# amberxie88/latent_diffusion_planning

Hardware: AMD Instinct MI355X
Metric: latent plans/sec (horizon=9, 100 DDIM steps) (higher is better)
Workload: dtype f32; 1 GPU; configs[1]: rm_lift planner ConditionalUnet1D (D=25, T=8, down_dims [256,512,1024]), 100-step DDIM, batch 256 synthetic latents per GPU, random-init weights, Philox noise, hipGraph-captured loop; plans_per_gpu=256, denoise_steps=100, sampler=ddim, graph=True, parallelism=dp1, ranks_seen_by_backend=1, backend=none, range_fallback=0, fp16_plane_launches=0

## Files before the change

### latent_diffusion_planning_amd/csrc/engine.hip

```cpp
#include "engine.hpp"
#include "sconv.hpp"
#include "t2pack.hpp"
#include "t4pack.hpp"
#include "version.h"

#include <algorithm>
#include <cmath>
#include <cstring>

namespace ldp {

void betas_squaredcos(int n, std::vector<float>& betas, std::vector<float>& alphas,
                             std::vector<float>& acp) {
  auto abar = [](double t) {
    const double c = std::cos((t + 0.008) / 1.008 * M_PI / 2.0);
    return c * c;
  };
  betas.resize(n);
  alphas.resize(n);
  acp.resize(n);
  float run = 1.0f;
  for (int i = 0; i < n; ++i) {
    const double b = std::min(1.0 - abar((double)(i + 1) / n) / abar((double)i / n), 0.999);
    betas[i] = (float)b;
// ... 145 lines not shown
            const uint16_t mm = f32_to_bf16_rne(r1);
            const float r2 = r1 - bf16_to_f32(mm);
            dst[0 * 512 + lane * 8 + e] = hh;
            dst[1 * 512 + lane * 8 + e] = mm;
            dst[2 * 512 + lane * 8 + e] = f32_to_bf16_rne(r2);
          }
      }
  return p;
}

bool fits_f16_planes(const float* w, size_t n) {
  for (size_t i = 0; i < n; ++i)
    if (!(std::fabs(w[i]) < 65504.0f)) return false;
  return true;
}

static int split_tile(int to, bool res_out) {
  if (to == 2) return 32;
  if (to == 8 || to == 4) return 16;
  return 0;
}

static bool split_tile_updown(int mode, int to, int cout) {
  const int bn = cout / 8;
  if (mode == MODE_DOWN) return (to == 4 && (bn == 32 || bn == 64)) || (to == 2 && bn == 64);
  if (mode == MODE_UP) return (to == 4 && bn == 64) || (to == 8 && (bn == 32 || bn == 64)) || (to == 16 && bn == 32);
  return false;
}

static bool t2_cs2_ok(const ldp_handle* h, int B, int cout) {
  const int wgs = ((B + 31) / 32) * 8;
  return h->opt.planner_split_cs2 && !h->opt.no_csplit && !h->safe_mode && cout % 512 == 0 && 2 * wgs <= h->n_cu && 8 * wgs >= 3 * h->n_cu;
}

static int split_tile_at(const ldp_handle* h, int B, int to, bool res_out, int cout) {
  int tile = split_tile(to, res_out);
  if (to == 16 && cout == 256 && !res_out && h->f16_planner() && h->opt.planner_split_t16) tile = 16;
  if (cout % 256 != 0 || (cout == 256 && (tile == 32 || h->opt.planner_split_c256 == 0))) return 0;
  if (tile == 32) {
    const int wgs = ((B + 31) / 32) * 8;
    const bool filled = wgs >= h->n_cu || h->opt.planner_split >= 2;
    if (!filled) {
      const bool cs2 = t2_cs2_ok(h, B, cout);
      const bool whole16 = h->opt.planner_split_t2res16 && h->opt.planner_split_t2all16 && h->f16_planner() && cout % 512 == 0 && B > 256;
      tile = (cs2 || whole16) ? 33 : 0;
    }
  }
  return tile;
}

int get_weight(ldp_handle* h, const std::string& path, const HostTensor** out,
               std::initializer_list<int64_t> shape) {
  auto it = h->weights.find(path);
  if (it == h->weights.end()) return fail(LDP_ESTATE, "weight '%s' was never set", path.c_str());
  const HostTensor& t = it->second;
  if (t.shape.size() != shape.size() || !std::equal(shape.begin(), shape.end(), t.shape.begin())) {
    std::string got, want;
    for (auto s : t.shape) got += std::to_string(s) + ",";
    for (auto s : shape) want += std::to_string(s) + ",";
    return fail(LDP_EINVAL, "weight '%s' has shape (%s) expected (%s)", path.c_str(), got.c_str(),
                want.c_str());
  }
  *out = &t;
  return LDP_OK;
}

static int upload_padded(DevBuf& dst, const float* src, int n, int n_p, float fill, hipStream_t s) {
  std::vector<float> tmp(n_p, fill);
  std::copy(src, src + n, tmp.begin());
  LDP_TRY(dst.alloc((size_t)n_p * 4));
  LDP_HIP(hipMemcpy(dst.p, tmp.data(), (size_t)n_p * 4, hipMemcpyHostToDevice));
  (void)s;
  return LDP_OK;
}

int make_conv(ldp_handle* h, const std::string& prefix, int nj, int cin, int cout, int cin_p,
              int cout_p, const char* gn_prefix, hipStream_t s, ConvW& out, int t_pos) {
  const HostTensor *k = nullptr, *b = nullptr;
  LDP_TRY(get_weight(h, prefix + "/kernel", &k, {nj, cin, cout}));
  LDP_TRY(get_weight(h, prefix + "/bias", &b, {cout}));
  out.t2s = nj == 5 && t2_shared(MODE_K5, t_pos, 0);
  out.t4s = nj == 5 && t4_shared(MODE_K5, t_pos, 0);
  std::vector<float> packed = out.t2s ? pack_conv_t2(k->data.data(), nullptr, cin, cout, cin_p, cout_p)
                            : out.t4s ? pack_conv_t4(k->data.data(), nullptr, cin, cout, cin_p, cout_p)
                                      : pack_conv(k->data.data(), nj, cin, cout, cin_p, cout_p);
  LDP_TRY(out.w.alloc(packed.size() * 4));
  LDP_HIP(hipMemcpy(out.w.p, packed.data(), packed.size() * 4, hipMemcpyHostToDevice));
  LDP_TRY(upload_padded(out.bias, b->data.data(), cout, cout_p, 0.f, s));
  out.nj = nj; out.cin = cin; out.cout = cout; out.cin_p = cin_p; out.cout_p = cout_p;
  out.has_gn = gn_prefix != nullptr;
  out.wsplit.release(); out.wsplit16.release(); out.wsplit16h.release(); out.wsplith.release();
  out.f16_refused = false;
  if (gn_prefix) {
    const HostTensor *gs = nullptr, *gb = nullptr;
    LDP_TRY(get_weight(h, std::string(gn_prefix) + "/scale", &gs, {cout}));
    LDP_TRY(get_weight(h, std::string(gn_prefix) + "/bias", &gb, {cout}));
    LDP_TRY(upload_padded(out.gn_scale, gs->data.data(), cout, cout_p, 1.f, s));
    LDP_TRY(upload_padded(out.gn_bias, gb->data.data(), cout, cout_p, 0.f, s));
  }
  return LDP_OK;
}

static int add_res_proj(ldp_handle* h, const std::string& conv_prefix, const std::string& prefix, int cin,
                        int cout, int cin_p, ConvW& c) {
  const HostTensor *k = nullptr, *b = nullptr, *kc = nullptr;
  LDP_TRY(get_weight(h, prefix + "/kernel", &k, {1, cin, cout}));
  LDP_TRY(get_weight(h, prefix + "/bias", &b, {cout}));
  LDP_TRY(get_weight(h, conv_prefix + "/kernel", &kc, {c.nj, cin, cout}));
  c.wsplit.release(); c.wsplit16.release(); c.wsplit16h.release(); c.wsplith.release();
  c.f16_refused = false;
  std::vector<float> packed;
  if (c.t2s) {
    packed = pack_conv_t2(kc->data.data(), k->data.data(), cin, cout, cin_p, c.cout_p);
  } else if (c.t4s) {
    packed = pack_conv_t4(kc->data.data(), k->data.data(), cin, cout, cin_p, c.cout_p);
  } else {
    std::vector<float> both(kc->data);
    both.insert(both.end(), k->data.begin(), k->data.end());
    packed = pack_conv(both.data(), c.nj + 1, cin, cout, cin_p, c.cout_p);
  }
  LDP_TRY(c.w.alloc(packed.size() * 4));
  LDP_HIP(hipMemcpy(c.w.p, packed.data(), packed.size() * 4, hipMemcpyHostToDevice));
  LDP_TRY(c.bres.alloc((size_t)cout * 4));
  LDP_HIP(hipMemcpy(c.bres.p, b->data.data(), (size_t)cout * 4, hipMemcpyHostToDevice));
  c.has_res = true;
  return LDP_OK;
}

static int round_up(int v, int m) { return (v + m - 1) / m * m; }

static int pick_plan(int mode, int to, int cout, int cin_total, int ca, bool res_out, ConvPlan& p,
                     int* cs_io = nullptr, int mb_want = 1, bool up_full_depth = false) {
  const int gw = cout >= 256 ? cout / 8 : 32;
  if (cs_io && *cs_io == 4) {
    const int qb = gw / 4;
    int ks4 = 0, cpi4 = 0;
    if (mode == MODE_K5) {
      if (to == 2 && qb == 32) { ks4 = 4; cpi4 = 2; }
      else if (to == 4 && qb == 16) { ks4 = 8; cpi4 = 1; }
      else if (to == 8 && qb == 16) { ks4 = 8; cpi4 = 1; }
      else if (to == 4 && qb == 32) { ks4 = 4; cpi4 = res_out ? 1 : 2; }
    }
    const int chunk4 = 16 * ks4 * cpi4;
    if (ks4 && cin_total % chunk4 == 0 && ca % chunk4 == 0) {
      p = ConvPlan{mode, to, qb / 16, ks4, cpi4, res_out ? 1 : 0};
      return LDP_OK;
    }
    *cs_io = 2;
  }
  if (cs_io && *cs_io == 2) {
    const int hb = gw / 2;
    int ks2 = 0, cpi2 = 0;
    if (mode == MODE_K5) {
      if (to == 8 && hb == 16) { ks2 = (cin_total % 128 == 0) ? 8 : 4; cpi2 = 1; }
      else if (to == 4 && hb == 32) { ks2 = 4; cpi2 = res_out ? 1 : 2; }
      else if (to == 2 && hb == 64) { ks2 = 2; cpi2 = res_out ? 2 : 4; }
      else if (to == 4 && hb == 16) { ks2 = 8; cpi2 = 1; }
      else if (to == 2 && hb == 32) { ks2 = 4; cpi2 = 2; }
      else if (to == 8 && hb == 32) { ks2 = 4; cpi2 = 1; }
      else if (to == 4 && hb == 64) { ks2 = 2; cpi2 = 2; }
      else if (to == 16 && hb == 16) { ks2 = 4; cpi2 = 1; }
    } else if (mode == MODE_DOWN) {
      if (to == 4 && hb == 16) { ks2 = 8; cpi2 = 1; }
      else if (to == 2 && hb == 32) { ks2 = 4; cpi2 = 2; }
      else if (to == 8 && hb == 16) { ks2 = 4; cpi2 = 1; }
    } else if (mode == MODE_UP) {
      if (to == 4 && hb == 32) { ks2 = 4; cpi2 = (cin_total % 256 == 0 && up_full_depth) ? 4 : 2; }
      else if (to == 8 && hb == 16) { ks2 = 8; cpi2 = (cin_total % 256 == 0 && up_full_depth) ? 2 : 1; }
      else if (to == 16 && hb == 16) { ks2 = 4; cpi2 = 1; }
    } else if (mode == MODE_P1) {
      if (to == 8 && hb == 16) { ks2 = 8; cpi2 = 1; }
    }
    const int chunk2 = 16 * ks2 * cpi2;
    if (ks2 && cin_total % chunk2 == 0 && ca % chunk2 == 0) {
      p = ConvPlan{mode, to, hb / 16, ks2, cpi2, res_out ? 1 : 0};
      return LDP_OK;
    }
    *cs_io = 1;
  }
  const int bn = gw;
  int nwn = bn / 16, ks = 0, cpi = 0;
  if (mode == MODE_K5) {
    if (to == 8 && bn == 32) { ks = (cin_total % 64 == 0) ? 4 : 2; cpi = 1; }
    else if (to == 8 && bn == 64) { ks = 2; cpi = 1; }
    else if (to == 4 && bn == 64) { ks = 2; cpi = 2; }
    else if (to == 4 && bn == 32) { ks = 4; cpi = res_out ? 1 : 2; }
    else if (to == 4 && bn == 128) { ks = 1; cpi = 2; }
    else if (to == 2 && bn == 128) { ks = 1; cpi = 4; }
    else if (to == 2 && bn == 64) { ks = 2; cpi = res_out ? 2 : 4; }
    else if (to == 16 && bn == 32) { ks = 2; cpi = 1; }
    else if (to == 2 && bn == 32) { ks = 4; cpi = 2; }
  } else if (mode == MODE_DOWN) {
    if (to == 4 && bn == 32) { ks = 4; cpi = 1; }
    else if (to == 2 && bn == 32) { ks = 4; cpi = 2; }
    else if (to == 2 && bn == 64) { ks = 2; cpi = 2; }
    else if (to == 8 && bn == 32) { ks = 2; cpi = 1; }
    else if (to == 4 && bn == 64) { ks = 2; cpi = 1; }
  } else if (mode == MODE_UP) {
// ... 1276 lines not shown
        if (rest == std::string(forms[f]) + "_" + tiles[t]) idx = f * 5 + t;
    if (idx < 0) return fail(LDP_EKEY, "unknown option '%s'", name);
    *value = h->stat_train_gemm[idx];
  }
  else if (n == "vae_no_conv_stats") *value = o.vae_no_conv_stats;
  else if (n == "vae_no_conv_in_stats") *value = o.vae_no_conv_in_stats;
  else if (n == "vae_split") *value = o.vae_split;
  else if (n == "vae_split_f16") *value = o.vae_split_f16;
  else if (n == "vae_split_gn_only") *value = o.vae_split_gn_only;
  else if (n == "vae_split_s2") *value = o.vae_split_s2;
  else if (n == "timeline_ptr") *value = o.timeline_ptr;
  else if (n == "idm_unfused") *value = o.idm_unfused;
  else if (n == "idm_rt_major") *value = o.idm_rt_major;
  else if (n == "idm_noring") *value = o.idm_noring;
  else if (n == "idm_stream") *value = o.idm_stream;
  else if (n == "by_sample") *value = o.by_sample;
  else if (n == "place2d") *value = o.place2d;
  else if (n == "idm_hs") *value = o.idm_hs;
  else if (n == "idm_f16") *value = o.idm_f16;
  else if (n == "idm_f16_min_rows") *value = o.idm_f16_min_rows;
  else if (n == "idm_f16_hs") *value = o.idm_f16_hs;
  else if (n == "train_small_wg") *value = o.train_small_wg;
  else if (n == "train_big") *value = o.train_big;
  else if (n == "train_split") *value = o.train_split;
  else if (n == "train_streams") *value = o.train_streams;
  else if (n == "train_intra_split") *value = o.train_intra_split;
  else if (n == "train_group_proj") *value = o.train_group_proj;
  else if (n == "train_gn4") *value = o.train_gn4;
  else if (n == "train_sides") *value = o.train_sides;
  else if (n == "train_fuse_reduce") *value = o.train_fuse_reduce;
  else if (n == "train_wg_target") *value = o.train_wg_target;
  else if (n == "dbg") *value = o.dbg;
  else if (n == "repeat") *value = o.repeat;
  else if (n == "t2_mb2") *value = o.t2_mb2;
  else if (n == "planner_split_t2all16") *value = o.planner_split_t2all16;
  else if (n == "planner_split_t2res16") *value = o.planner_split_t2res16;
  else if (n == "planner_split_8w") *value = o.planner_split_8w;
  else if (n == "safe_mode") *value = h->safe_mode ? 1 : 0;
  else if (n == "range_fallback") *value = h->range_fallback ? 1 : 0;
  else if (n == "range_faults_seen") *value = h->range_faults_seen;
  else if (n == "any_debug") *value = o.any_debug() ? 1 : 0;
  else if (n == "faults_seen") *value = h->faults_seen;
  else if (n == "n_cu") *value = h->n_cu;
  else if (n == "graphs") *value = (int64_t)h->graphs.size();
  else if (n == "graph_cap") *value = h->graph_cap;
  else if (n == "graphs_captured") *value = h->graphs_captured;
  else if (n == "graphs_evicted") *value = h->graphs_evicted;
  else return fail(LDP_EKEY, "unknown option '%s'", name);
  return LDP_OK;
}

int ldp_philox_raw(uint64_t seed, uint64_t elem0, uint32_t step, uint32_t stream_id, uint32_t* out_dev,
                   int64_t n, void* stream) {
  if (!out_dev || n <= 0) return fail(LDP_EINVAL, "bad argument");
  return philox_raw_launch(seed, elem0, step, stream_id, out_dev, n, (hipStream_t)stream);
}

int ldp_philox_normal(uint64_t seed, uint64_t elem0, uint32_t step, uint32_t stream_id, float* out_dev,
                      int64_t n, void* stream) {
  if (!out_dev || n <= 0) return fail(LDP_EINVAL, "bad argument");
  return philox_normal_launch(seed, elem0, step, stream_id, out_dev, n, (hipStream_t)stream);
}

int ldp_launch_count(ldp_handle* h, int32_t which, int64_t* launches) {
  if (!h || !launches) return fail(LDP_EINVAL, "bad argument");
  *launches = which == 0 ? h->last_conv_launches : h->last_total_launches;
  return LDP_OK;
}

static int prim_conv(int mode, const float* x, const float* kernel_host, const float* bias_host,
                     const float* gs, const float* gb, const float* film, float* y, int B, int t_in,
                     int cin, int cout, void* stream) {
  if (!x || !kernel_host || !bias_host || !y || B <= 0) return fail(LDP_EINVAL, "bad argument");
  hipStream_t s = (hipStream_t)stream;
  const int nj = mode_taps(mode);
  const int to = mode == MODE_DOWN ? t_in / 2 : mode == MODE_UP ? t_in * 2 : t_in;
  if (cout % 128 != 0) return fail(LDP_EINVAL, "Cout must be a multiple of 128 (8 groups x 16)");
  const int cin_p = round_up(cin, 32);
  ConvPlan p;
  LDP_TRY(pick_plan(mode, to, cout, cin_p, cin_p, false, p));
  const int cin_pp = round_up(cin_p, p.chunk());
  if (cin_pp != cin_p) LDP_TRY(pick_plan(mode, to, cout, cin_pp, cin_pp, false, p));
  std::vector<float> packed = t2_shared(mode, to, 0) ? pack_conv_t2(kernel_host, nullptr, cin, cout, cin_pp, cout)
                            : t4_shared(mode, to, 0) ? pack_conv_t4(kernel_host, nullptr, cin, cout, cin_pp, cout)
                                                     : pack_conv(kernel_host, nj, cin, cout, cin_pp, cout);
  DevBuf dw, db, dgs, dgb, dx, dfg, dft;
  LDP_TRY(upload(dw, packed.data(), packed.size() * 4, s));
  LDP_TRY(upload(db, bias_host, (size_t)cout * 4, s));
  ConvArgs a{};
  if (gs) {
    LDP_TRY(upload(dgs, gs, (size_t)cout * 4, s));
    LDP_TRY(upload(dgb, gb, (size_t)cout * 4, s));
    a.flags |= EP_GN;
  }
  const float* xin = x;
  if (cin_pp != cin) {
    LDP_TRY(dx.alloc((size_t)B * t_in * cin_pp * 4));
    LDP_TRY(pad_rows_launch(x, dx.f(), (int64_t)B * t_in, cin, cin_pp, s));
    xin = dx.f();
  }
  if (film) {
    LDP_TRY(dft.alloc((size_t)2 * cout * 4));
    LDP_HIP(hipMemsetAsync(dft.p, 0, (size_t)2 * cout * 4, s));
    a.film_t = dft.f(); a.film_g = film; a.film_stride = 2 * cout; a.flags |= EP_FILM;
  }
  a.xa = xin; a.ca = cin_pp; a.w = dw.f(); a.bias = db.f();
  a.gn_scale = dgs.f(); a.gn_bias = dgb.f();
  a.out = y; a.B = B; a.cout = cout; a.k = 0; a.rows_valid = B * to;
  const int r = tconv_launch(p, a, s);
  if (r != 0) return fail(r == -100 ? LDP_EINVAL : LDP_EHIP, "primitive conv launch failed (%d)", r);
  LDP_HIP(hipStreamSynchronize(s));
  return LDP_OK;
}

int ldp_conv1d_gn_mish_film_f32(const float* x, const float* kernel_host, const float* bias_host,
                                const float* gn_scale_host, const float* gn_bias_host,
                                const float* film, float* y, int32_t B, int32_t T, int32_t Cin,
                                int32_t Cout, void* stream) {
  if (!gn_scale_host || !gn_bias_host) return fail(LDP_EINVAL, "GroupNorm parameters required");
  return prim_conv(MODE_K5, x, kernel_host, bias_host, gn_scale_host, gn_bias_host, film, y, B, T, Cin,
                   Cout, stream);
}

int ldp_downsample1d_f32(const float* x, const float* kernel_host, const float* bias_host, float* y,
                         int32_t B, int32_t T, int32_t C, void* stream) {
  if (T % 2) return fail(LDP_EINVAL, "T must be even");
  return prim_conv(MODE_DOWN, x, kernel_host, bias_host, nullptr, nullptr, nullptr, y, B, T, C, C, stream);
}

int ldp_upsample1d_f32(const float* x, const float* kernel_host, const float* bias_host, float* y,
                       int32_t B, int32_t T, int32_t C, void* stream) {
  return prim_conv(MODE_UP, x, kernel_host, bias_host, nullptr, nullptr, nullptr, y, B, T, C, C, stream);
}

}
```

### latent_diffusion_planning_amd/csrc/t4pack.hpp

```cpp
#pragma once
#include <cstddef>
#include <vector>

namespace ldp {

inline void t4_combine(const float w[5], float out[9]) {
  const double w0 = w[0], w1 = w[1], w2 = w[2], w3 = w[3], w4 = w[4];
  const double a = w4 - w2, ap = w0 - w2;
  out[0] = w[2];
  out[1] = (float)(w3 - w2);
  out[2] = (float)(w1 - w2);
  out[3] = (float)a;
  out[4] = (float)(-w3 - a);
  out[5] = (float)(w3 - w1 - a);
  out[6] = (float)ap;
  out[7] = (float)(w1 - w3 - ap);
  out[8] = (float)(-w1 - ap);
}

inline std::vector<float> pack_conv_t4(const float* w, const float* proj, int cin, int cout, int cin_p, int cout_p) {
  const int nchunk = cin_p / 16, nblk = cout_p / 16, ns = proj ? 10 : 9;
  std::vector<float> p((size_t)nchunk * ns * nblk * 256, 0.0f);
  for (int gc = 0; gc < nchunk; ++gc)
    for (int nb = 0; nb < nblk; ++nb)
      for (int lane = 0; lane < 64; ++lane) {
        const int kq = lane >> 4, n = lane & 15;
        const int co = nb * 16 + n;
        for (int s = 0; s < 4; ++s) {
          const int ci = gc * 16 + 4 * kq + s;
          if (ci >= cin || co >= cout) continue;
          float taps[5], v[9];
          for (int j = 0; j < 5; ++j) taps[j] = w[((size_t)j * cin + ci) * cout + co];
          t4_combine(taps, v);
          for (int sl = 0; sl < ns; ++sl)
            p[(((size_t)gc * ns + sl) * nblk + nb) * 256 + lane * 4 + s] = sl < 9 ? v[sl] : proj[(size_t)ci * cout + co];
        }
      }
  return p;
}

}
```

### latent_diffusion_planning_amd/csrc/tconv.hpp

```cpp
#pragma once
#include <hip/hip_runtime.h>
#include <stdint.h>
#include <type_traits>

#pragma clang fp contract(off)

#ifndef LDP_W_NT
#define LDP_W_NT 0
#endif
#ifndef LDP_SPLIT_NPROD
#define LDP_SPLIT_NPROD 6
#endif
#ifndef LDP_S16_LF
#define LDP_S16_LF 100
#endif
#ifndef LDP_F16_MINW
#define LDP_F16_MINW 2
#endif
#ifndef LDP_RANGE_GUARD
#define LDP_RANGE_GUARD 1
#endif
#ifndef LDP_KERNARG_TOUCH
#define LDP_KERNARG_TOUCH 1
#endif
// ... 59 lines not shown
  unsigned int* fault;
  int h_out, w_tiles, h_in, w_in;
  int ca_real;
  int by_sample;
  float* stats_part;
  int sb_qs;
  unsigned long long* tl;
};

#ifdef LDP_ABLATE
#define LDP_ABL(bit) ((a.dbg & (bit)) != 0)
#else
#define LDP_ABL(bit) (false)
#endif

#ifdef LDP_TIMELINE
#define LDP_TL(i)                                                                                         \
  do {                                                                                                    \
    if (a.tl) {                                                                                           \
      const unsigned long long t_ = (i) == 0 ? ldp_t_entry : __builtin_amdgcn_s_memtime();                \
      if (lane == 0)                                                                                      \
        a.tl[((size_t)(blockIdx.x + gridDim.x * (blockIdx.y + gridDim.y * blockIdx.z)) * 16 + wave) * 8 + (i)] = t_; \
    }                                                                                                     \
  } while (0)
#else
#define LDP_TL(i) do { } while (0)
#endif

__host__ __device__ constexpr int mode_taps(int mode) {
  return mode == MODE_K5 ? 5 : (mode == MODE_DOWN || mode == MODE_K3H || mode == MODE_K3S) ? 3
       : mode == MODE_UP ? 4 : 1;
}
__host__ __device__ constexpr bool mode_2d(int mode) { return mode == MODE_K3H || mode == MODE_K3S; }
__host__ __device__ constexpr int mode_ti(int mode, int to) {
  return mode == MODE_DOWN ? 2 * to : mode == MODE_UP ? to / 2 : mode == MODE_K3H ? to + 2
       : mode == MODE_K3S ? 2 * to + 2 : to;
}
__host__ __device__ constexpr int tap_src(int mode, int to, int j) {
  if (mode == MODE_K5) return to + j - 2;
  if (mode == MODE_DOWN || mode == MODE_K3S) return 2 * to + j;
  if (mode == MODE_K3H) return to + j;
  if (mode == MODE_UP) {
    const int q = to >> 1;
    if ((to & 1) == 0) return j == 0 ? q - 1 : (j == 2 ? q : -1);
    return j == 1 ? q : (j == 3 ? q + 1 : -1);
  }
  return j == 0 ? to : -1;
}
__host__ __device__ constexpr int tap_dst(int mode, int to_n, int ti, int j) {
  for (int to = 0; to < to_n; ++to)
    if (tap_src(mode, to, j) == ti) return to;
  return -1;
}
__host__ __device__ constexpr bool tap_used(int mode, int to_n, int j) {
  const int ti_n = mode_ti(mode, to_n);
  for (int to = 0; to < to_n; ++to) {
    const int ti = tap_src(mode, to, j);
    if (ti >= 0 && ti < ti_n) return true;
  }
  return false;
}
__host__ __device__ constexpr int valid_pairs(int mode, int to_n) {
  const int ti_n = mode_ti(mode, to_n);
  int n = 0;
  for (int to = 0; to < to_n; ++to)
    for (int j = 0; j < mode_taps(mode); ++j) {
      const int ti = tap_src(mode, to, j);
      if (ti >= 0 && ti < ti_n) ++n;
    }
  return n;
}

#ifndef LDP_T2_DIRECT
#define LDP_T2_DIRECT 0
#endif
__host__ __device__ constexpr bool t2_shared(int mode, int to_n, int split) {
  return !LDP_T2_DIRECT && mode == MODE_K5 && to_n == 2 && split == 0;
}
constexpr int T2_SLOTS = 3;

#ifndef LDP_T4_DIRECT
#define LDP_T4_DIRECT 0
#endif
__host__ __device__ constexpr bool t4_shared(int mode, int to_n, int split) {
  return !LDP_T4_DIRECT && mode == MODE_K5 && to_n == 4 && split == 0;
}
constexpr int T4_SLOTS = 9;
__host__ __device__ constexpr int conv_products(int mode, int to_n, int split) {
  return t2_shared(mode, to_n, split) ? T2_SLOTS : t4_shared(mode, to_n, split) ? T4_SLOTS : valid_pairs(mode, to_n);
}

__device__ __forceinline__ int swz(int row, int slot) { return slot ^ ((4 - (row >> 2)) & 3); }

#ifndef LDP_EPILOGUE_IEEE
#define LDP_EPILOGUE_IEEE 0
#endif
__device__ __forceinline__ float mish_f(float x) {
#if LDP_EPILOGUE_IEEE
  const float e = expf(fminf(x, 20.0f));
  const float n = e * (e + 2.0f);
  return x * (n / (n + 2.0f));
#else
  const float e = __builtin_amdgcn_exp2f(fminf(x, 20.0f) * 1.4426950408889634f);
  const float n = e * (e + 2.0f);
  return x * (n * __builtin_amdgcn_rcpf(n + 2.0f));
#endif
}

template <int CTRL, int ROW_MASK>
__device__ __forceinline__ float dpp_add(float v) {
  return v + __int_as_float(__builtin_amdgcn_update_dpp(0, __float_as_int(v), CTRL, ROW_MASK, 0xF, false));
}
__device__ __forceinline__ float wave_sum(float v) {
  v = dpp_add<0xB1, 0xF>(v);
  v = dpp_add<0x4E, 0xF>(v);
  v = dpp_add<0x114, 0xF>(v);
  v = dpp_add<0x118, 0xF>(v);
  v = dpp_add<0x142, 0xA>(v);
  v = dpp_add<0x143, 0xC>(v);
  return __int_as_float(__builtin_amdgcn_readlane(__float_as_int(v), 63));
}

__device__ __forceinline__ unsigned long long granule_pack(unsigned int tag, float v) {
  const unsigned int b = __float_as_uint(v);
  return ((unsigned long long)(tag ^ b) << 32) | b;
}
typedef unsigned int u32x4_t __attribute__((ext_vector_type(4)));
constexpr int AUX_SC1 = 16;

__device__ __forceinline__ bool granule_ok(unsigned long long g, unsigned int tag) {
  return ((unsigned int)(g >> 32) ^ (unsigned int)g) == tag;
}

__device__ __forceinline__ void philox4x32_10(uint64_t seed, uint64_t elem, uint32_t step, uint32_t stream,
                                              uint32_t (&out)[4]) {
  uint32_t c0 = (uint32_t)elem, c1 = (uint32_t)(elem >> 32), c2 = step, c3 = stream;
  uint32_t k0 = (uint32_t)seed, k1 = (uint32_t)(seed >> 32);
#pragma unroll
  for (int r = 0; r < 10; ++r) {
    const uint64_t p0 = (uint64_t)0xD2511F53u * c0;
    const uint64_t p1 = (uint64_t)0xCD9E8D57u * c2;
    const uint32_t n0 = (uint32_t)(p1 >> 32) ^ c1 ^ k0;
    const uint32_t n1 = (uint32_t)p1;
    const uint32_t n2 = (uint32_t)(p0 >> 32) ^ c3 ^ k1;
    const uint32_t n3 = (uint32_t)p0;
    c0 = n0; c1 = n1; c2 = n2; c3 = n3;
    k0 += 0x9E3779B9u; k1 += 0xBB67AE85u;
  }
  out[0] = c0; out[1] = c1; out[2] = c2; out[3] = c3;
}

__device__ __forceinline__ float philox_normal(uint64_t seed, uint64_t elem, uint32_t step,
                                               uint32_t stream) {
  uint32_t w[4];
  philox4x32_10(seed, elem, step, stream, w);
  const float u1 = ((float)(w[0] >> 8) + 0.5f) * (1.0f / 16777216.0f);
  const float u2 = ((float)(w[1] >> 8) + 0.5f) * (1.0f / 16777216.0f);
  return sqrtf(-2.0f * logf(u1)) * cosf(6.28318530717958647692f * u2);
}

__host__ __device__ constexpr int mode_flag_mask(int mode) {
  return mode == MODE_K5 ? (EP_GN | EP_FILM | EP_RESIN)
       : mode == MODE_P1 ? (EP_RESIN | EP_RELU | EP_STEP | EP_EPSOUT)
       : mode_2d(mode) ? EP_RESIN : 0;
}
__host__ __device__ constexpr int mode_flag_forced(int mode) { return mode == MODE_K5 ? EP_GN : 0; }

template <int MODE, int TO, int NWN, int KS, int CPI, int MB = 1, int SPLIT = 0>
struct TConvCfg {
  static constexpr int TI = mode_ti(MODE, TO);
// ... 180 lines not shown
  int st_mask[mode_2d(MODE) ? C::NLD : 1];
#pragma unroll
  for (int i = 0; i < C::NLD; ++i) {
    const int idx = tid + i * NT;
    const int q = idx & 3;
    const int cc = (idx >> 2) % NC;
    const int rr = (idx / (4 * NC)) & 15;
    const int tm = idx / (64 * NC);
    const int tt = tm % TI, mb = tm / TI;
    st_cc[i] = cc * 16 + q * 4;
    const int bb = (b0 + mb * 16 + rr) < a.B ? (b0 + mb * 16 + rr) : (a.B - 1);
    st_goff[i] = bb * TI + tt;
    st_loff[i] = (((mb * TI + tt) * NC + cc) * 16 + rr) * 16 + swz(rr, q) * 4;
    if constexpr (S32) st_loff[i] = (((tt * NC + cc) * C::NPL) * 64 + (q >> 1) * 32 + mb * 16 + rr) * 4 + (q & 1) * 2;
    if constexpr (S16) st_loff[i] = ((((mb * TI + tt) * (NC / 2) + (cc >> 1)) * C::NPL) * 64 + ((cc & 1) * 2 + (q >> 1)) * 16 + rr) * 4 + (q & 1) * 2;
    if (mode_2d(MODE)) {
      const int wt = bb % a.w_tiles, hh = (bb / a.w_tiles) % a.h_out, n = bb / (a.w_tiles * a.h_out);
      const int w = MODE == MODE_K3H ? wt * TO - 1 + tt : 2 * wt * TO + tt;
      const int h0 = MODE == MODE_K3H ? hh - 1 : 2 * hh;
      const bool wok = w >= 0 && w < a.w_in;
      int m = 0;
#pragma unroll
      for (int dh = 0; dh < 3; ++dh) m |= (wok && h0 + dh >= 0 && h0 + dh < a.h_in) ? (1 << dh) : 0;
      st_mask[i] = m;
      st_goff[i] = (n * a.h_in + h0) * a.w_in + w;
    }
  }

  f32x4 xst[C::NLD];
  auto stage_load = [&](auto pass_tag, int it) {
    constexpr int SI0 = T4P ? decltype(pass_tag)::value * (C::NLD / 2) : 0, SI1 = T4P ? SI0 + C::NLD / 2 : C::NLD;
    const int c0 = it * C::CH_IT;
    if (mode_2d(MODE)) {
      const int dh = c0 / a.ca, cbase = c0 - dh * a.ca;
#pragma unroll
      for (int i = 0; i < C::NLD; ++i) {
        const bool ok = (st_mask[i] >> dh) & 1;
        const int pix = ok ? st_goff[i] + dh * a.w_in : 0;
        const f32x4 v = *reinterpret_cast<const f32x4*>(a.xa + (size_t)pix * a.ca + cbase + st_cc[i]);
        xst[i] = ok ? v : f32x4{0.f, 0.f, 0.f, 0.f};
      }
      return;
    }
    const bool second = (c0 >= a.ca);
    const float* base = second ? a.xb : a.xa;
    const int cw = second ? a.cb : a.ca;
    const int cbase = second ? c0 - a.ca : c0;
    const int creal = a.ca_real > 0 ? a.ca_real : 0x7fffffff;
    const int stride = a.ca_real > 0 ? a.ca_real : cw;
#pragma unroll
    for (int i = SI0; i < SI1; ++i) {
      const bool ok = (cbase + st_cc[i]) < creal;
      xst[i] = *reinterpret_cast<const f32x4*>(base + (size_t)st_goff[i] * stride + (ok ? cbase + st_cc[i] : 0));
    }
  };
  auto stage_store = [&](auto pass_tag, float* buf) {
    constexpr int SI0 = T4P ? decltype(pass_tag)::value * (C::NLD / 2) : 0, SI1 = T4P ? SI0 + C::NLD / 2 : C::NLD;
    if constexpr (C::F16) {
#pragma unroll
      for (int i = 0; i < C::NLD; ++i) {
        uint2 ph, pl;
        split4h(xst[i], ph, pl);
        *reinterpret_cast<uint2*>(buf + st_loff[i]) = ph;
        *reinterpret_cast<uint2*>(buf + st_loff[i] + 256) = pl;
      }
      return;
    }
    if constexpr (SPLIT) {
#pragma unroll
      for (int i = 0; i < C::NLD; ++i) {
        uint2 ph, pm, pl;
        split4(xst[i], ph, pm, pl);
        *reinterpret_cast<uint2*>(buf + st_loff[i]) = ph;
        *reinterpret_cast<uint2*>(buf + st_loff[i] + 256) = pm;
        *reinterpret_cast<uint2*>(buf + st_loff[i] + 512) = pl;
      }
      return;
    }
#pragma unroll
    for (int i = SI0; i < SI1; ++i) *reinterpret_cast<f32x4*>(buf + st_loff[i]) = xst[i];
  };

  constexpr bool SKIPZ = MODE == MODE_K5 && RES_OUT && SPLIT == 0 && TO >= 8 && KS > 1;
  constexpr int NJR = T2S ? T2_SLOTS : T4S ? T4_SLOTS : NJ;
  constexpr int NJW = NJR + (RES_OUT ? 1 : 0);
  constexpr int NJB = T4S ? T4_SLOTS : NJ;
  constexpr int NSTEP = S16 ? CPI / 2 : 1;
  constexpr int WCH = S16 ? 1 : CPI;
  constexpr int RN = RES_OUT ? WCH : 1;
  constexpr int WPL = SPLIT ? C::NPL : 1;
  f32x4 wb0[NJB][WCH * WPL], wb1[NJB][WCH * WPL];
  f32x4 rb0[RN * WPL], rb1[RN * WPL];
  auto wload = [&](int it, f32x4 (&b)[NJB][WCH * WPL], f32x4 (&rb)[RN * WPL]) {
#pragma unroll
    for (int ci = 0; ci < WCH; ++ci) {
      const int gc = S16 ? (it / NSTEP) * (NC / 2) + ks * NSTEP + (it % NSTEP) : it * NC + ks * CPI + ci;
#pragma unroll
      for (int j = 0; j < NJB; ++j) {
        if constexpr (SPLIT) {
          if (tap_used(MODE, TO, j)) {
#pragma unroll
            for (int pl = 0; pl < WPL; ++pl) {
              const size_t off = ((((size_t)gc * NJW + j) * nblk_total + nblk) * WPL + pl) * 256 + lane * 4;
              b[j][ci * WPL + pl] = *reinterpret_cast<const f32x4*>(a.w + off);
            }
          }
        } else
        if (T4S || tap_used(MODE, TO, j)) {
          const size_t off = (((size_t)gc * NJW + (T2S ? j - 1 : j)) * nblk_total + nblk) * 256 + lane * 4;
          b[j][ci] = (LDP_W_NT && KWS) ? __builtin_nontemporal_load(reinterpret_cast<const f32x4*>(a.w + off))
                                       : *reinterpret_cast<const f32x4*>(a.w + off);
        }
      }
      if constexpr (RES_OUT && SPLIT) {
#pragma unroll
        for (int pl = 0; pl < WPL; ++pl) {
          const size_t off = ((((size_t)gc * NJW + NJ) * nblk_total + nblk) * WPL + pl) * 256 + lane * 4;
          rb[ci * WPL + pl] = *reinterpret_cast<const f32x4*>(a.w + off);
        }
      } else
      if (RES_OUT) {
        const size_t off = (((size_t)gc * NJW + NJR) * nblk_total + nblk) * 256 + lane * 4;
        rb[ci] = (LDP_W_NT && KWS) ? __builtin_nontemporal_load(reinterpret_cast<const f32x4*>(a.w + off))
                                   : *reinterpret_cast<const f32x4*>(a.w + off);
      }
    }
  };

  f32x16 acc32[S32 ? TO : 1], racc32[S32 && RES_OUT ? TO : 1];
  f32x16 acc32_lo[S32 && C::F16 ? TO : 1], racc32_lo[S32 && C::F16 && RES_OUT ? TO : 1];
  if constexpr (S32 && C::F16) {
#pragma unroll
    for (int t = 0; t < TO; ++t)
#pragma unroll
      for (int i = 0; i < 16; ++i) acc32_lo[t][i] = 0.f;
#pragma unroll
    for (int t = 0; t < (RES_OUT ? TO : 1); ++t)
#pragma unroll
      for (int i = 0; i < 16; ++i) racc32_lo[t][i] = 0.f;
  }
  if constexpr (S32) {
#pragma unroll
    for (int t = 0; t < TO; ++t)
#pragma unroll
      for (int i = 0; i < 16; ++i) acc32[t][i] = 0.f;
#pragma unroll
    for (int t = 0; t < (RES_OUT ? TO : 1); ++t)
#pragma unroll
      for (int i = 0; i < 16; ++i) racc32[t][i] = 0.f;
  }
  auto iteration = [&](auto pass_tag, auto last_tag, int it, f32x4 (&bc)[NJB][WCH * WPL], f32x4 (&rc)[RN * WPL], f32x4 (&bl)[NJB][WCH * WPL],
                       f32x4 (&rl)[RN * WPL]) {
    constexpr bool LAST = decltype(last_tag)::value;
    constexpr int PASS = decltype(pass_tag)::value;
    float* xcur = smem + (it & 1) * C::XT;
    float* xnext = smem + ((it + 1) & 1) * C::XT;
    const int itn = LDP_ABL(256) ? it0 : (LAST || (it + 1) < nit) ? it + 1 : it;
    if (!LAST) {
      if (!(SPLIT && LDP_ABL(2048))) stage_load(pass_tag, itn);
      if (!S16 && !(SPLIT && LDP_ABL(1024))) wload(itn, bl, rl);
    }
    if constexpr (S16) {
      constexpr int NPAIR = valid_pairs(MODE, TO) + (RES_OUT ? TO : 0);
      constexpr int NUSED = (tap_used(MODE, TO, 0) ? 1 : 0) + (NJ > 1 && tap_used(MODE, TO, 1) ? 1 : 0) + (NJ > 2 && tap_used(MODE, TO, 2) ? 1 : 0) +
                            (NJ > 3 && tap_used(MODE, TO, 3) ? 1 : 0) + (NJ > 4 && tap_used(MODE, TO, 4) ? 1 : 0);
      constexpr int NPL = C::NPL;
      constexpr int NWL = (NUSED + (RES_OUT ? 1 : 0)) * NPL;
      constexpr int NMFMA = (C::F16 ? 3 : LDP_SPLIT_NPROD) * NPAIR * MB;
      constexpr int NREAD = MB * TI * NPL;
      constexpr int AHEAD = MB * (TI > 2 ? 2 : TI) * NPL;
      auto step = [&](auto pc_tag, f32x4 (&wc)[NJB][WCH * WPL], f32x4 (&rcur)[RN * WPL], f32x4 (&wn)[NJB][WCH * WPL], f32x4 (&rnext)[RN * WPL]) {
        constexpr int pc = decltype(pc_tag)::value;
        constexpr bool PREF = pc + 1 < NSTEP || !LAST;
        if (PREF && !LDP_ABL(1024)) wload(pc + 1 < NSTEP ? it * NSTEP + pc + 1 : itn * NSTEP, wn, rnext);
        f32x4 asp[MB][TI][NPL];
#pragma unroll
        for (int ti = 0; ti < TI; ++ti) {
#pragma unroll
          for (int m = 0; m < MB; ++m)
#pragma unroll
            for (int pl = 0; pl < NPL; ++pl)
              asp[m][ti][pl] = *reinterpret_cast<const f32x4*>(xcur + (((((m * TI + ti) * (NC / 2) + ks * NSTEP + pc) * NPL + pl) * 64 + lane) * 4));
        }
        if constexpr (C::F16) {
          constexpr int FA[3] = {1, 0, 0}, FB[3] = {0, 1, 0};
#pragma unroll
          for (int ti = 0; ti < TI; ++ti) {
#pragma unroll
            for (int pi = 0; pi < 3; ++pi) {
#pragma unroll
              for (int j = 0; j <= NJ; ++j) {
// ... 99 lines not shown
#pragma unroll
          for (int to = 0; to < TO; ++to) {
            const int ti = tap_src(MODE, to, j);
            if (ti >= 0 && ti < TI) pair(&asp[ti][ci][0], &bc[j][ci * WPL], acc32[to], acc32_lo[C::F16 ? to : 0]);
          }
      if constexpr (RES_OUT) {
#pragma unroll
        for (int ci = 0; ci < CPI; ++ci)
#pragma unroll
          for (int to = 0; to < TO; ++to) pair(&asp[to][ci][0], &rc[ci * WPL], racc32[to], racc32_lo[C::F16 ? to : 0]);
      }
      {
        constexpr int NUSED = (tap_used(MODE, TO, 0) ? 1 : 0) + (NJ > 1 && tap_used(MODE, TO, 1) ? 1 : 0) + (NJ > 2 && tap_used(MODE, TO, 2) ? 1 : 0) +
                              (NJ > 3 && tap_used(MODE, TO, 3) ? 1 : 0) + (NJ > 4 && tap_used(MODE, TO, 4) ? 1 : 0);
        constexpr int NLOADS = LAST ? 0 : C::NLD + (NUSED + (RES_OUT ? 1 : 0)) * CPI * C::NPL;
        constexpr int NMFMA = CPI * (C::F16 ? 3 : 6) * (valid_pairs(MODE, TO) + (RES_OUT ? TO : 0));
        constexpr int MPL = NMFMA / (NLOADS > 0 ? NLOADS : 1) > 0 ? NMFMA / (NLOADS > 0 ? NLOADS : 1) : 1;
#pragma unroll
        for (int i = 0; i < TI * CPI * C::NPL; ++i) __builtin_amdgcn_sched_group_barrier(0x100, 1, 0);
#pragma unroll
        for (int i = 0; i < NLOADS; ++i) {
          __builtin_amdgcn_sched_group_barrier(0x020, 1, 0);
          __builtin_amdgcn_sched_group_barrier(0x008, MPL, 0);
        }
        if (NMFMA - NLOADS * MPL > 0) __builtin_amdgcn_sched_group_barrier(0x008, NMFMA - NLOADS * MPL, 0);
      }
      if (!LAST) stage_store(pass_tag, xnext);
      __syncthreads();
      return;
    }
    f32x4 areg[MB][TI][CPI];
#pragma unroll
    for (int m = 0; m < MB; ++m)
#pragma unroll
      for (int ti = 0; ti < TI; ++ti)
#pragma unroll
        for (int ci = 0; ci < CPI; ++ci)
          areg[m][ti][ci] = *reinterpret_cast<const f32x4*>(
              xcur + (((m * TI + ti) * NC + ks * CPI + ci) * 16 + r) * 16 + swz(r, kq) * 4);

    const bool dead_slice = SKIPZ && a.ca_real > 0 && (it * C::CH_IT + ks * CPI * 16) >= a.ca_real;
    if constexpr (T2S) {
      f32x4 asum[MB][CPI];
#pragma unroll
      for (int m = 0; m < MB; ++m)
#pragma unroll
        for (int ci = 0; ci < CPI; ++ci) asum[m][ci] = areg[m][0][ci] + areg[m][1][ci];
#pragma unroll
      for (int ci = 0; ci < CPI; ++ci) {
#pragma unroll
        for (int s = 0; s < 4; ++s) {
          const bool odd = T2S2 && (ci & 1);
#pragma unroll
          for (int m = 0; m < MB; ++m) {
            f32x4& d = odd ? sacc_b[m] : sacc[m];
            d = __builtin_amdgcn_mfma_f32_16x16x4f32(asum[m][ci][s], bc[1][ci][s], d, 0, 0, 0);
          }
#pragma unroll
          for (int m = 0; m < MB; ++m) {
            f32x4& d = odd ? acc_b[m][0] : acc[m][0];
            d = __builtin_amdgcn_mfma_f32_16x16x4f32(areg[m][1][ci][s], bc[2][ci][s], d, 0, 0, 0);
          }
#pragma unroll
          for (int m = 0; m < MB; ++m) {
            f32x4& d = odd ? acc_b[m][1] : acc[m][1];
            d = __builtin_amdgcn_mfma_f32_16x16x4f32(areg[m][0][ci][s], bc[3][ci][s], d, 0, 0, 0);
          }
          if (RES_OUT) {
#pragma unroll
            for (int to = 0; to < TO; ++to)
#pragma unroll
              for (int m = 0; m < MB; ++m)
                racc[m][to] = __builtin_amdgcn_mfma_f32_16x16x4f32(areg[m][to][ci][s], rc[ci][s], racc[m][to], 0, 0, 0);
          }
        }
      }
    } else
    if constexpr (T4S) {
      f32x4 tit[T4F ? MB : 1][T4F ? T4_SLOTS : 1];
#pragma unroll
      for (int m = 0; m < (T4F ? MB : 1); ++m)
#pragma unroll
        for (int k = 0; k < (T4F ? T4_SLOTS : 1); ++k) tit[m][k] = f32x4{0.f, 0.f, 0.f, 0.f};
#pragma unroll
      for (int ci = 0; ci < CPI; ++ci) {
        f32x4 af[MBE][T4_SLOTS];
#pragma unroll
        for (int mm = 0; mm < MBE; ++mm) {
          const int m = T4P ? PASS : mm;
          const f32x4 x0 = areg[m][0][ci], x1 = areg[m][1][ci], x2 = areg[m][2][ci], x3 = areg[m][3][ci];
          const f32x4 u0 = x0 + x2, u1 = x1 + x3;
          af[mm][0] = u0 + u1; af[mm][1] = u1; af[mm][2] = u0;
          af[mm][3] = x2 + x3; af[mm][4] = x3; af[mm][5] = x2;
          af[mm][6] = x0 + x1; af[mm][7] = x1; af[mm][8] = x0;
        }
#pragma unroll
        for (int s = 0; s < 4; ++s) {
#pragma unroll
          for (int k = 0; k < T4_SLOTS; ++k) {
#pragma unroll
            for (int m = 0; m < MBE; ++m) {
              f32x4& d = T4F ? tit[T4F ? m : 0][T4F ? k : 0] : tacc[T4F ? 0 : m][T4F ? 0 : k];
              d = __builtin_amdgcn_mfma_f32_16x16x4f32(af[m][k][s], bc[k][ci][s], d, 0, 0, 0);
            }
          }
          if (RES_OUT) {
#pragma unroll
            for (int to = 0; to < TO; ++to)
#pragma unroll
              for (int m = 0; m < MB; ++m)
                racc[m][to] = __builtin_amdgcn_mfma_f32_16x16x4f32(areg[m][to][ci][s], rc[ci][s], racc[m][to], 0, 0, 0);
          }
        }
      }
      if constexpr (T4F) {
#pragma unroll
        for (int m = 0; m < MB; ++m) {
          const f32x4 se0 = tit[m][0] + tit[m][1], se1 = tit[m][0] + tit[m][2];
          acc[m][0] = acc[m][0] + ((se0 + tit[m][3]) + tit[m][4]);
          acc[m][1] = acc[m][1] + ((se1 + tit[m][3]) + tit[m][5]);
          acc[m][2] = acc[m][2] + ((se0 + tit[m][6]) + tit[m][7]);
          acc[m][3] = acc[m][3] + ((se1 + tit[m][6]) + tit[m][8]);
        }
      }
    } else
    if (!dead_slice) {
#pragma unroll
    for (int ci = 0; ci < CPI; ++ci) {
#pragma unroll
      for (int s = 0; s < 4; ++s) {
#pragma unroll
        for (int j = 0; j < NJ; ++j) {
#pragma unroll
          for (int to = 0; to < TO; ++to) {
            const int ti = tap_src(MODE, to, j);
            if (ti >= 0 && ti < TI) {
#pragma unroll
              for (int m = 0; m < MB; ++m)
                acc[m][to] = __builtin_amdgcn_mfma_f32_16x16x4f32(areg[m][ti][ci][s], bc[j][ci][s],
                                                                  acc[m][to], 0, 0, 0);
            }
          }
        }
        if (RES_OUT) {
#pragma unroll
          for (int to = 0; to < TO; ++to)
#pragma unroll
            for (int m = 0; m < MB; ++m)
              racc[m][to] = __builtin_amdgcn_mfma_f32_16x16x4f32(areg[m][to][ci][s], rc[ci][s],
                                                                 racc[m][to], 0, 0, 0);
        }
      }
    }
    }
    if (LAST) {
#pragma unroll
      for (int i = 0; i < MBE * TI * CPI; ++i) __builtin_amdgcn_sched_group_barrier(0x100, 1, 0);
    } else {
      constexpr int NUSED = (tap_used(MODE, TO, 0) ? 1 : 0) + (NJ > 1 && tap_used(MODE, TO, 1) ? 1 : 0) +
                            (NJ > 2 && tap_used(MODE, TO, 2) ? 1 : 0) + (NJ > 3 && tap_used(MODE, TO, 3) ? 1 : 0) +
                            (NJ > 4 && tap_used(MODE, TO, 4) ? 1 : 0);
      constexpr int NLOADS = NLDE + ((T4S ? T4_SLOTS : NUSED) + (RES_OUT ? 1 : 0)) * CPI;
      constexpr int NMFMA = MBE * CPI * 4 * (conv_products(MODE, TO, SPLIT) + (RES_OUT ? TO : 0));
      constexpr int MPL = NMFMA / NLOADS > 0 ? NMFMA / NLOADS : 1;
#pragma unroll
      for (int i = 0; i < MBE * TI * CPI; ++i) __builtin_amdgcn_sched_group_barrier(0x100, 1, 0);
#pragma unroll
      for (int i = 0; i < NLOADS; ++i) {
        __builtin_amdgcn_sched_group_barrier(0x020, 1, 0);
        __builtin_amdgcn_sched_group_barrier(0x008, MPL, 0);
      }
      if (NMFMA - NLOADS * MPL > 0) __builtin_amdgcn_sched_group_barrier(0x008, NMFMA - NLOADS * MPL, 0);
      __builtin_amdgcn_sched_group_barrier(0x200, NLDE, 0);
    }
    if (!LAST) stage_store(pass_tag, xnext);
    __syncthreads();
  };

#define LDP_TCONV_PASS(pass_tag) \
  stage_load(pass_tag, it0); \
  wload(S16 ? it0 * NSTEP : it0, wb0, rb0); \
  stage_store(pass_tag, smem + (it0 & 1) * C::XT); \
  __syncthreads(); \
  LDP_TL(1); \
  if (mode_2d(MODE) && !S16) { \
    for (int it = it0; it < nit; it += 2) { \
      iteration(pass_tag, std::false_type{}, it, wb0, rb0, wb1, rb1); \
      if (it + 1 < nit) iteration(pass_tag, std::false_type{}, it + 1, wb1, rb1, wb0, rb0); \
    } \
  } else { \
    int it = it0; \
    if constexpr (S16 && NSTEP % 2 == 0) { \
      for (; it + 1 < nit; ++it) iteration(pass_tag, std::false_type{}, it, wb0, rb0, wb1, rb1); \
      iteration(pass_tag, std::true_type{}, it, wb0, rb0, wb1, rb1); \
    } else { \
    for (; it + 2 < nit; it += 2) { \
      iteration(pass_tag, std::false_type{}, it, wb0, rb0, wb1, rb1); \
      iteration(pass_tag, std::false_type{}, it + 1, wb1, rb1, wb0, rb0); \
    } \
    if (it + 2 == nit) { \
      iteration(pass_tag, std::false_type{}, it, wb0, rb0, wb1, rb1); \
      iteration(pass_tag, std::true_type{}, it + 1, wb1, rb1, wb0, rb0); \
    } else if (it + 1 == nit) { \
      iteration(pass_tag, std::true_type{}, it, wb0, rb0, wb1, rb1); \
    } \
    } \
  }
  auto t4_combine_pass = [&](auto pass_tag) {
  if constexpr (T4S && !T4F) {
    constexpr int PASS = decltype(pass_tag)::value;
#pragma unroll
    for (int mm = 0; mm < MBE; ++mm) {
      const int m = T4P ? PASS : mm;
      const f32x4 se0 = tacc[mm][0] + tacc[mm][1], se1 = tacc[mm][0] + tacc[mm][2];
      acc[m][0] = (se0 + tacc[mm][3]) + tacc[mm][4];
      acc[m][1] = (se1 + tacc[mm][3]) + tacc[mm][5];
      acc[m][2] = (se0 + tacc[mm][6]) + tacc[mm][7];
      acc[m][3] = (se1 + tacc[mm][6]) + tacc[mm][8];
#pragma unroll
      for (int k = 0; k < T4_SLOTS; ++k) tacc[mm][k] = f32x4{0.f, 0.f, 0.f, 0.f};
    }
  }
  };
  {
    using pass0 = std::integral_constant<int, 0>;
    LDP_TCONV_PASS(pass0{})
    t4_combine_pass(pass0{});
  }
  if constexpr (T4P) {
    using pass1 = std::integral_constant<int, 1>;
    LDP_TCONV_PASS(pass1{})
    t4_combine_pass(pass1{});
  }
#undef LDP_TCONV_PASS

  if constexpr (T2S) {
#pragma unroll
    for (int m = 0; m < MB; ++m) {
      if constexpr (T2S2) {
        sacc[m] = sacc[m] + sacc_b[m];
        acc[m][0] = acc[m][0] + acc_b[m][0];
        acc[m][1] = acc[m][1] + acc_b[m][1];
      }
      acc[m][0] = sacc[m] + acc[m][0];
      acc[m][1] = sacc[m] + acc[m][1];
// ... 440 lines not shown
```

Baseline: 5823 plans/s.

## Derive T4 Winograd-style weight slots on device from raw taps instead of packed slots

With the new default (LDP_T4_PACKED=0), T4-shared K5 convolutions now load only the 5 raw tap weights per chunk and compute the 9 combined weight slots in registers, double-buffered one chunk ahead. This cuts weight memory traffic and register staging from 9 slots to 5 taps, at the cost of extra VALU subtractions interleaved with the MFMAs. Inline asm barriers pin the derivation order. The old precomputed-slot packing stays available behind the macro, with a float derivation matching the device arithmetic.

Result: no change. 5861 plans/s, median of 6 (+0.7%).

```diff
diff --git a/latent_diffusion_planning_amd/csrc/engine.hip b/latent_diffusion_planning_amd/csrc/engine.hip
--- a/latent_diffusion_planning_amd/csrc/engine.hip
+++ b/latent_diffusion_planning_amd/csrc/engine.hip
@@ -251,7 +251,7 @@
   out.t2s = nj == 5 && t2_shared(MODE_K5, t_pos, 0);
   out.t4s = nj == 5 && t4_shared(MODE_K5, t_pos, 0);
   std::vector<float> packed = out.t2s ? pack_conv_t2(k->data.data(), nullptr, cin, cout, cin_p, cout_p)
-                            : out.t4s ? pack_conv_t4(k->data.data(), nullptr, cin, cout, cin_p, cout_p)
+                            : out.t4s && LDP_T4_PACKED ? pack_conv_t4(k->data.data(), nullptr, cin, cout, cin_p, cout_p, t4_derive)
                                       : pack_conv(k->data.data(), nj, cin, cout, cin_p, cout_p);
   LDP_TRY(out.w.alloc(packed.size() * 4));
   LDP_HIP(hipMemcpy(out.w.p, packed.data(), packed.size() * 4, hipMemcpyHostToDevice));
@@ -281,8 +281,8 @@
   std::vector<float> packed;
   if (c.t2s) {
     packed = pack_conv_t2(kc->data.data(), k->data.data(), cin, cout, cin_p, c.cout_p);
-  } else if (c.t4s) {
-    packed = pack_conv_t4(kc->data.data(), k->data.data(), cin, cout, cin_p, c.cout_p);
+  } else if (c.t4s && LDP_T4_PACKED) {
+    packed = pack_conv_t4(kc->data.data(), k->data.data(), cin, cout, cin_p, c.cout_p, t4_derive);
   } else {
     std::vector<float> both(kc->data);
     both.insert(both.end(), k->data.begin(), k->data.end());
@@ -1725,7 +1725,7 @@
   const int cin_pp = round_up(cin_p, p.chunk());
   if (cin_pp != cin_p) LDP_TRY(pick_plan(mode, to, cout, cin_pp, cin_pp, false, p));
   std::vector<float> packed = t2_shared(mode, to, 0) ? pack_conv_t2(kernel_host, nullptr, cin, cout, cin_pp, cout)
-                            : t4_shared(mode, to, 0) ? pack_conv_t4(kernel_host, nullptr, cin, cout, cin_pp, cout)
+                            : t4_shared(mode, to, 0) && LDP_T4_PACKED ? pack_conv_t4(kernel_host, nullptr, cin, cout, cin_pp, cout, t4_derive)
                                                      : pack_conv(kernel_host, nj, cin, cout, cin_pp, cout);
   DevBuf dw, db, dgs, dgb, dx, dfg, dft;
   LDP_TRY(upload(dw, packed.data(), packed.size() * 4, s));
diff --git a/latent_diffusion_planning_amd/csrc/t4pack.hpp b/latent_diffusion_planning_amd/csrc/t4pack.hpp
--- a/latent_diffusion_planning_amd/csrc/t4pack.hpp
+++ b/latent_diffusion_planning_amd/csrc/t4pack.hpp
@@ -18,7 +18,17 @@
   out[8] = (float)(-w1 - ap);
 }
 
-inline std::vector<float> pack_conv_t4(const float* w, const float* proj, int cin, int cout, int cin_p, int cout_p) {
+inline void t4_derive(const float w[5], float out[9]) {
+  const float w0 = w[0], w1 = w[1], w2 = w[2], w3 = w[3], w4 = w[4];
+  const float s1 = w3 - w2, s2 = w1 - w2, s3 = w4 - w2, s6 = w0 - w2;
+  const float s4 = (-s1) - w4, s8 = (-s2) - w0;
+  const float t = s1 - s2;
+  const float s5 = t - s3, s7 = (-t) - s6;
+  out[0] = w2; out[1] = s1; out[2] = s2; out[3] = s3; out[4] = s4; out[5] = s5; out[6] = s6; out[7] = s7; out[8] = s8;
+}
+
+template <class Combine>
+inline std::vector<float> pack_conv_t4(const float* w, const float* proj, int cin, int cout, int cin_p, int cout_p, Combine combine) {
   const int nchunk = cin_p / 16, nblk = cout_p / 16, ns = proj ? 10 : 9;
   std::vector<float> p((size_t)nchunk * ns * nblk * 256, 0.0f);
   for (int gc = 0; gc < nchunk; ++gc)
@@ -31,12 +41,15 @@
           if (ci >= cin || co >= cout) continue;
           float taps[5], v[9];
           for (int j = 0; j < 5; ++j) taps[j] = w[((size_t)j * cin + ci) * cout + co];
-          t4_combine(taps, v);
+          combine(taps, v);
           for (int sl = 0; sl < ns; ++sl)
             p[(((size_t)gc * ns + sl) * nblk + nb) * 256 + lane * 4 + s] = sl < 9 ? v[sl] : proj[(size_t)ci * cout + co];
         }
       }
   return p;
 }
+inline std::vector<float> pack_conv_t4(const float* w, const float* proj, int cin, int cout, int cin_p, int cout_p) {
+  return pack_conv_t4(w, proj, cin, cout, cin_p, cout_p, t4_combine);
+}
 
 }
diff --git a/latent_diffusion_planning_amd/csrc/tconv.hpp b/latent_diffusion_planning_amd/csrc/tconv.hpp
--- a/latent_diffusion_planning_amd/csrc/tconv.hpp
+++ b/latent_diffusion_planning_amd/csrc/tconv.hpp
@@ -165,10 +165,30 @@
 #ifndef LDP_T4_DIRECT
 #define LDP_T4_DIRECT 0
 #endif
+#ifndef LDP_T4_PACKED
+#define LDP_T4_PACKED 0
+#endif
 __host__ __device__ constexpr bool t4_shared(int mode, int to_n, int split) {
   return !LDP_T4_DIRECT && mode == MODE_K5 && to_n == 4 && split == 0;
 }
 constexpr int T4_SLOTS = 9;
+template <class V>
+__device__ __forceinline__ void t4_slots(const V& w0, const V& w1, const V& w2, const V& w3, const V& w4, V (&o)[T4_SLOTS]) {
+  const V s1 = w3 - w2, s2 = w1 - w2, s3 = w4 - w2, s6 = w0 - w2;
+  const V s4 = (-s1) - w4, s8 = (-s2) - w0;
+  const V t = s1 - s2;
+  const V s5 = t - s3, s7 = (-t) - s6;
+  o[0] = w2; o[1] = s1; o[2] = s2; o[3] = s3; o[4] = s4; o[5] = s5; o[6] = s6; o[7] = s7; o[8] = s8;
+}
+template <bool PACKED, class V, int NJB, int W>
+__device__ __forceinline__ void t4_chunk_slots(const V (&b)[NJB][W], int ci, V (&o)[T4_SLOTS]) {
+  if constexpr (PACKED) {
+#pragma unroll
+    for (int k = 0; k < T4_SLOTS; ++k) o[k] = b[k < NJB ? k : 0][ci];
+  } else {
+    t4_slots(b[0][ci], b[1][ci], b[2][ci], b[3][ci], b[4 < NJB ? 4 : 0][ci], o);
+  }
+}
 __host__ __device__ constexpr int conv_products(int mode, int to_n, int split) {
   return t2_shared(mode, to_n, split) ? T2_SLOTS : t4_shared(mode, to_n, split) ? T4_SLOTS : valid_pairs(mode, to_n);
 }
@@ -515,9 +535,10 @@
   };
 
   constexpr bool SKIPZ = MODE == MODE_K5 && RES_OUT && SPLIT == 0 && TO >= 8 && KS > 1;
-  constexpr int NJR = T2S ? T2_SLOTS : T4S ? T4_SLOTS : NJ;
+  constexpr bool T4K = T4S && LDP_T4_PACKED;
+  constexpr int NJR = T2S ? T2_SLOTS : T4K ? T4_SLOTS : NJ;
   constexpr int NJW = NJR + (RES_OUT ? 1 : 0);
-  constexpr int NJB = T4S ? T4_SLOTS : NJ;
+  constexpr int NJB = T4K ? T4_SLOTS : NJ;
   constexpr int NSTEP = S16 ? CPI / 2 : 1;
   constexpr int WCH = S16 ? 1 : CPI;
   constexpr int RN = RES_OUT ? WCH : 1;
@@ -539,7 +560,7 @@
             }
           }
         } else
-        if (T4S || tap_used(MODE, TO, j)) {
+        if (T4K || tap_used(MODE, TO, j)) {
           const size_t off = (((size_t)gc * NJW + (T2S ? j - 1 : j)) * nblk_total + nblk) * 256 + lane * 4;
           b[j][ci] = (LDP_W_NT && KWS) ? __builtin_nontemporal_load(reinterpret_cast<const f32x4*>(a.w + off))
                                        : *reinterpret_cast<const f32x4*>(a.w + off);
@@ -805,6 +826,9 @@
       for (int m = 0; m < (T4F ? MB : 1); ++m)
 #pragma unroll
         for (int k = 0; k < (T4F ? T4_SLOTS : 1); ++k) tit[m][k] = f32x4{0.f, 0.f, 0.f, 0.f};
+      f32x4 wd[CPI > 1 ? 2 : 1][T4_SLOTS];
+      if constexpr (!T4K) asm("" : "+v"(bc[2][0]) : "v"(areg[T4P ? PASS : 0][0][0][0]));
+      t4_chunk_slots<T4K>(bc, 0, wd[0]);
 #pragma unroll
       for (int ci = 0; ci < CPI; ++ci) {
         f32x4 af[MBE][T4_SLOTS];
@@ -824,7 +848,7 @@
 #pragma unroll
             for (int m = 0; m < MBE; ++m) {
               f32x4& d = T4F ? tit[T4F ? m : 0][T4F ? k : 0] : tacc[T4F ? 0 : m][T4F ? 0 : k];
-              d = __builtin_amdgcn_mfma_f32_16x16x4f32(af[m][k][s], bc[k][ci][s], d, 0, 0, 0);
+              d = __builtin_amdgcn_mfma_f32_16x16x4f32(af[m][k][s], wd[ci & 1][k][s], d, 0, 0, 0);
             }
           }
           if (RES_OUT) {
@@ -833,6 +857,10 @@
 #pragma unroll
               for (int m = 0; m < MB; ++m)
                 racc[m][to] = __builtin_amdgcn_mfma_f32_16x16x4f32(areg[m][to][ci][s], rc[ci][s], racc[m][to], 0, 0, 0);
+          }
+          if (s == 0 && ci + 1 < CPI) {
+            if constexpr (!T4K) asm("" : "+v"(bc[2][ci + 1 < CPI ? ci + 1 : 0]) : "v"(T4F ? tit[0][0] : tacc[0][0]));
+            t4_chunk_slots<T4K>(bc, ci + 1, wd[(ci + 1) & 1]);
           }
         }
       }
@@ -883,7 +911,7 @@
       constexpr int NUSED = (tap_used(MODE, TO, 0) ? 1 : 0) + (NJ > 1 && tap_used(MODE, TO, 1) ? 1 : 0) +
                             (NJ > 2 && tap_used(MODE, TO, 2) ? 1 : 0) + (NJ > 3 && tap_used(MODE, TO, 3) ? 1 : 0) +
                             (NJ > 4 && tap_used(MODE, TO, 4) ? 1 : 0);
-      constexpr int NLOADS = NLDE + ((T4S ? T4_SLOTS : NUSED) + (RES_OUT ? 1 : 0)) * CPI;
+      constexpr int NLOADS = NLDE + ((T4K ? T4_SLOTS : NUSED) + (RES_OUT ? 1 : 0)) * CPI;
       constexpr int NMFMA = MBE * CPI * 4 * (conv_products(MODE, TO, SPLIT) + (RES_OUT ? TO : 0));
       constexpr int MPL = NMFMA / NLOADS > 0 ? NMFMA / NLOADS : 1;
 #pragma unroll
```
